# tvlabs/edge264

Hardware: AMD Instinct MI355X
Metric: 1080p frames/s/GPU (bit-exact YUV) + achieved HBM GB/s vs 8 TB/s peak (higher is better)
Workload: dtype u8

## Files before the change

edge264_amd/csrc/e264_dev.h:

```cpp
#ifndef E264_DEV_H
#define E264_DEV_H
#include <stdint.h>
#include <stddef.h>
#include "../../include/edge264_cmd.h"
#include "e264_kernels.h"

#ifndef E264_DEV
#define E264_DEV __device__ __forceinline__
#endif
#ifndef E264_AS_GLOBAL
#define E264_AS_GLOBAL __attribute__((address_space(1)))
#define E264_AS_CONST __attribute__((address_space(4)))
#endif

#ifndef E264_HOST_INTRINSICS
#define E264_FIRST(x) __builtin_amdgcn_readfirstlane(x)
#define E264_BALLOT(x) __ballot(x)
#define E264_ANY(x) __any(x)
#define E264_WG_SYNC() __syncthreads()
#define E264_WG_OR(x) __syncthreads_or(x)
#define E264_SLEEP() __builtin_amdgcn_s_sleep(1)
#define E264_FENCE_ACQUIRE() __builtin_amdgcn_fence(__ATOMIC_ACQUIRE, "workgroup")
#define E264_FENCE_RELEASE() __builtin_amdgcn_fence(__ATOMIC_RELEASE, "workgroup")
#define E264_PROGRESS_STORE(p, v) __hip_atomic_store((p), (v), __ATOMIC_RELAXED, __HIP_MEMORY_SCOPE_WORKGROUP)
#define E264_PROGRESS_LOAD(p) __hip_atomic_load((p), __ATOMIC_RELAXED, __HIP_MEMORY_SCOPE_WORKGROUP)
#define E264_ROW_TAKE(p) __hip_atomic_fetch_add((p), 1, __ATOMIC_RELAXED, __HIP_MEMORY_SCOPE_WORKGROUP)
#define E264_TASK_TAKE(p) atomicAdd((p), 1)
#define E264_SETPRIO(n) __builtin_amdgcn_s_setprio(n)
#define E264_PIN(...) asm volatile("" :: __VA_ARGS__)
#define E264_EMU_DBKP_RAW(L, f, a0)
#define E264_EMU_DBK_STEP(filtered)
#endif
#define E264_MAX_ROWS 1056

namespace {

#if defined(E264_DBK_TIMELINE) || defined(E264_PHASE_TIMING)
__device__ unsigned long long g_phase[32];
__device__ unsigned long long g_timeline[128];
#endif
#ifdef E264_PHASE_TIMING
#define PH_DECL unsigned long long ph_t = __builtin_amdgcn_s_memtime(), ph_acc[14] = {0, 0, 0, 0, 0, 0, 0, 0, 0, 0, 0, 0, 0, 0}
#define PH(k) do { __builtin_amdgcn_sched_barrier(0); unsigned long long t_ = __builtin_amdgcn_s_memtime(); __builtin_amdgcn_s_waitcnt(0xc07f); __builtin_amdgcn_sched_barrier(0); ph_acc[k] += t_ - ph_t; ph_t = t_; } while (0)
#define PH_FLUSH(lane) do { if ((lane) == 0) for (int k_ = 0; k_ < 14; k_++) atomicAdd(&g_phase[k_], ph_acc[k_]); } while (0)
#define PH_FLUSH_DBK(lane) do { if ((lane) == 0) for (int k_ = 0; k_ < 14; k_++) atomicAdd(&g_phase[16 + k_], ph_acc[k_]); } while (0)
#define PH_PARAMS , unsigned long long &ph_t, unsigned long long (&ph_acc)[14]
#define PH_ARGS , ph_t, ph_acc
#else
#define PH_DECL
#define PH(k)
#define PH_FLUSH(lane)
#define PH_FLUSH_DBK(lane)
#define PH_PARAMS
#define PH_ARGS
#endif

E264_DEV int clip3i(int lo, int hi, int v) { return min(max(v, lo), hi); }
E264_DEV int clip255(int v) { return min(max(v, 0), 255); }
E264_DEV int sat16(int v) { return min(max(v, -32768), 32767); }
E264_DEV int w16(int v) { return (int)(int16_t)v; }
#ifdef E264_ABL_NOBH
#define E264_ABL_BH && false
#else
#define E264_ABL_BH
#endif
#ifndef E264_LUMA_PACKED
#define E264_LUMA_PACKED 1
#endif
typedef uint8_t E264_AS_GLOBAL gu8;
typedef uint32_t E264_AS_GLOBAL gu32;
typedef uint16_t E264_AS_GLOBAL gu16;
typedef uint32_t E264_AS_GLOBAL __attribute__((aligned(1))) gu32u;
typedef uint32_t v4u __attribute__((ext_vector_type(4)));
typedef uint32_t v2u __attribute__((ext_vector_type(2)));
typedef v4u E264_AS_GLOBAL __attribute__((aligned(4))) gv4u;
typedef v2u E264_AS_GLOBAL __attribute__((aligned(4))) gv2u;
typedef uint32_t v3u __attribute__((ext_vector_type(3)));
typedef v3u E264_AS_GLOBAL __attribute__((aligned(4))) gv3u;
typedef int16_t E264_AS_GLOBAL gi16;
typedef const E264FrameHdr E264_AS_CONST *chdr_t;
typedef const E264SliceParams E264_AS_CONST *cslice_t;
typedef const E264Mb E264_AS_CONST *cmb_t;
typedef const E264Motion E264_AS_GLOBAL *gmotion_t;
typedef const uint8_t E264_AS_CONST *cu8p;
typedef uint8_t *generic_u8p;
typedef const generic_u8p E264_AS_GLOBAL *gdpb_t;
#ifndef E264_HOST_INTRINSICS
E264_DEV int lane_id() { return (int)(threadIdx.x & 63); }
E264_DEV void wave_sync()
{
	__builtin_amdgcn_fence(__ATOMIC_ACQ_REL, "wavefront");
	__builtin_amdgcn_wave_barrier();
}
#endif
#define lds_load_relaxed(p) E264_PROGRESS_LOAD(p)

__constant__ uint8_t c_BX[16] = {0, 4, 0, 4, 8, 12, 8, 12, 0, 4, 0, 4, 8, 12, 8, 12};
__constant__ uint8_t c_BY[16] = {0, 0, 4, 4, 0, 0, 4, 4, 8, 8, 12, 12, 8, 8, 12, 12};
E264_DEV int BXf(int k) { return ((k & 1) << 2) | ((k & 4) << 1); }
E264_DEV int BYf(int k) { return ((k & 2) << 1) | ((k & 8)); }
E264_DEV int blk_of(int bx, int by) { return (by >> 1) * 8 + (bx >> 1) * 4 + (by & 1) * 2 + (bx & 1); }

E264_DEV int na_byte(uint64_t t, int m) { return (int)(t >> (8 * m)) & 255; }
#define NA4_0 0x12100e0d0b0aull
#define NA4_1 0x1d1917141210ull
E264_DEV int norm4(int m, int pos)
{
	int i = pos >> 2, j = pos & 3;
	const int a = na_byte(NA4_0, m), b = na_byte(NA4_1, m), c = na_byte(0x171412100e0dull, m);
	return (i & j & 1) ? b : ((i | j) & 1) ? c : a;
}
E264_DEV int norm8(int m, int pos)
{
	int i = pos >> 3, j = pos & 7, k;
	const int v0 = na_byte(0x24201c1a1614ull, m), v1 = na_byte(0x201c19171312ull, m), v2 = na_byte(0x3a332d2a2320ull, m);
	const int v3 = na_byte(0x221e1a181513ull, m), v4 = na_byte(0x2e2823211c19ull, m), v5 = na_byte(0x2b26211f1a18ull, m);
	if ((i & 3) == 0 && (j & 3) == 0) k = v0;
	else if (i & j & 1) k = v1;
	else if ((i & 3) == 2 && (j & 3) == 2) k = v2;
	else if (((i & 3) == 0 && (j & 1)) || ((i & 1) && (j & 3) == 0)) k = v3;
	else if (((i & 3) == 0 && (j & 3) == 2) || ((i & 3) == 2 && (j & 3) == 0)) k = v4;
	else k = v5;
	return k;
}

__constant__ uint8_t c_alpha[52] = {0, 0, 0, 0, 0, 0, 0, 0, 0, 0, 0, 0, 0, 0, 0, 0, 4, 4, 5, 6, 7, 8, 9, 10, 12, 13, 15, 17, 20, 22, 25, 28,
	32, 36, 40, 45, 50, 56, 63, 71, 80, 90, 101, 113, 127, 144, 162, 182, 203, 226, 255, 255};
__constant__ uint8_t c_beta[52] = {0, 0, 0, 0, 0, 0, 0, 0, 0, 0, 0, 0, 0, 0, 0, 0, 2, 2, 2, 3, 3, 3, 3, 4, 4, 4, 6, 6, 7, 7, 8, 8,
	9, 9, 10, 10, 11, 11, 12, 12, 13, 13, 14, 14, 15, 15, 16, 16, 17, 17, 18, 18};
__constant__ uint8_t c_tc0[3][52] = {
	{0, 0, 0, 0, 0, 0, 0, 0, 0, 0, 0, 0, 0, 0, 0, 0, 0, 0, 0, 0, 0, 0, 0, 1, 1, 1, 1, 1, 1, 1, 1, 1, 1, 2, 2, 2, 2, 3, 3, 3, 4, 4, 4, 5, 6, 6, 7, 8, 9, 10, 11, 13},
	{0, 0, 0, 0, 0, 0, 0, 0, 0, 0, 0, 0, 0, 0, 0, 0, 0, 0, 0, 0, 0, 1, 1, 1, 1, 1, 1, 1, 1, 1, 1, 2, 2, 2, 2, 3, 3, 3, 4, 4, 5, 5, 6, 7, 8, 8, 10, 11, 12, 13, 15, 17},
	{0, 0, 0, 0, 0, 0, 0, 0, 0, 0, 0, 0, 0, 0, 0, 0, 0, 1, 1, 1, 1, 1, 1, 1, 1, 1, 1, 2, 2, 2, 2, 3, 3, 3, 4, 4, 4, 5, 6, 6, 7, 8, 9, 10, 11, 13, 14, 16, 18, 20, 23, 25}};

#ifndef E264_HOST_INTRINSICS
E264_DEV uint32_t v_perm(uint32_t hi, uint32_t lo, uint32_t sel) { return __builtin_amdgcn_perm(hi, lo, sel); }
E264_DEV uint32_t v_alignbyte(uint32_t hi, uint32_t lo, uint32_t sh) { return __builtin_amdgcn_alignbyte(hi, lo, sh); }
E264_DEV uint32_t v_alignbit(uint32_t hi, uint32_t lo, uint32_t sh) { return __builtin_amdgcn_alignbit(hi, lo, sh); }
E264_DEV uint32_t v_lerp_u8(uint32_t a, uint32_t b, uint32_t c) { return __builtin_amdgcn_lerp(a, b, c); }
E264_DEV int mul24(int a, int b) { return a * b; }
E264_DEV uint32_t v_sat_pk_u8_i16(uint32_t v)
{
	uint32_t r;
	asm("v_sat_pk_u8_i16 %0, %1" : "=v"(r) : "v"(v));
	return r;
}
#endif
typedef short s16x2 __attribute__((ext_vector_type(2)));
E264_DEV s16x2 as_s2(uint32_t v) { return __builtin_bit_cast(s16x2, v); }
E264_DEV uint32_t as_u(s16x2 v) { return __builtin_bit_cast(uint32_t, v); }
template <int I>
E264_DEV s16x2 pair_at(uint32_t hi, uint32_t lo)
{
	return as_s2(v_perm(hi, lo, 0x0c000c00u | (uint32_t)I | (uint32_t)(I + 1) << 16));
}
E264_DEV void pairs9(const uint32_t w[3], s16x2 Q[8])
{
	Q[0] = pair_at<0>(w[1], w[0]); Q[1] = pair_at<1>(w[1], w[0]); Q[2] = pair_at<2>(w[1], w[0]); Q[3] = pair_at<3>(w[1], w[0]);
	Q[4] = pair_at<0>(w[2], w[1]); Q[5] = pair_at<1>(w[2], w[1]); Q[6] = pair_at<2>(w[2], w[1]); Q[7] = pair_at<3>(w[2], w[1]);
}
E264_DEV s16x2 tap6u(s16x2 a, s16x2 b, s16x2 c, s16x2 d, s16x2 e, s16x2 f)
{
	const s16x2 k5 = {-5, -5}, k20 = {20, 20};
	const s16x2 af = as_s2(as_u(a) + as_u(f)), be = as_s2(as_u(b) + as_u(e)), cd = as_s2(as_u(c) + as_u(d));
	return be * k5 + (cd * k20 + af);
}
E264_DEV s16x2 tap6u16(s16x2 a, s16x2 b, s16x2 c, s16x2 d, s16x2 e, s16x2 f)
{
	const s16x2 k5 = {-5, -5}, k20 = {20, 20};
	const s16x2 af = as_s2(as_u(a) + as_u(f) + 0x00100010u), be = as_s2(as_u(b) + as_u(e)), cd = as_s2(as_u(c) + as_u(d));
	return be * k5 + (cd * k20 + af);
}
E264_DEV uint32_t packus4(s16x2 lo, s16x2 hi) { return v_perm(v_sat_pk_u8_i16(as_u(hi)), v_sat_pk_u8_i16(as_u(lo)), 0x05040100u); }
E264_DEV s16x2 tap6p(s16x2 a, s16x2 b, s16x2 c, s16x2 d, s16x2 e, s16x2 f)
{
	const s16x2 k5 = {5, 5}, k20 = {20, 20};
	return (a + f) - (b + e) * k5 + (c + d) * k20;
}
E264_DEV s16x2 centre6p(s16x2 t0, s16x2 t1, s16x2 t2, s16x2 t3, s16x2 t4, s16x2 t5)
{
	const s16x2 s2 = {2, 2}, s6 = {6, 6}, r32 = {32, 32}, z = {0, 0}, m = {255, 255};
	const s16x2 af = t0 + t5, be = t1 + t4, cd = t2 + t3;
	const s16x2 x1 = af - be;
	const s16x2 x2 = (x1 >> s2) + (cd - be);
	const s16x2 x3 = (x2 >> s2) + cd;
	return __builtin_elementwise_min(__builtin_elementwise_max((x3 + r32) >> s6, z), m);
}
E264_DEV s16x2 half5p(s16x2 v)
{
	const s16x2 s5 = {5, 5}, r16 = {16, 16}, z = {0, 0}, m = {255, 255};
	return __builtin_elementwise_min(__builtin_elementwise_max((v + r16) >> s5, z), m);
}
#ifndef E264_HOST_INTRINSICS
E264_DEV uint32_t any_u32() { uint32_t v; asm("" : "=v"(v)); return v; }
#else
E264_DEV uint32_t any_u32() { return 0xa55a5aa5u; }
#endif
E264_DEV uint32_t mot_nmv(uint32_t sub) { return 0x4221u >> (sub * 4) & 15u; }
struct DbkpQuad { v2u a, b; uint32_t c; };
E264_DEV DbkpQuad dbkp_quad_any() { return (DbkpQuad){(v2u){any_u32(), any_u32()}, (v2u){any_u32(), any_u32()}, any_u32()}; }
E264_DEV bool dbkp_list_has(uint32_t h, int l) { return (E264_MOT_UNI(h, l) | (h >> (4 * l) & 15u)) != 0; }
E264_DEV uint32_t dbkp_part_off(uint32_t mot_off, uint32_t h, int l)
{
	uint32_t n0 = 0;
#pragma unroll
	for (int k = 0; k < 4; k++)
		n0 += E264_MOT_USED(h, k) ? 4 + 4 * mot_nmv(E264_MOT_SUB(h, k)) : 0;
	return l ? mot_off + (E264_MOT_UNI(h, 0) ? 8 : n0) : mot_off;
}
E264_DEV DbkpQuad dbkp_fetch_quad(const gu8 *motion, uint32_t pa, uint32_t sub)
{
	DbkpQuad F;
	F.a = *(const gv2u *)(motion + pa);
	F.b = *(const gv2u *)(motion + (pa + (sub == 3 ? 8u : sub ? 4u : 0u)));
	F.c = *(const gu32 *)(motion + (pa + (sub == 3 ? 16u : 0u)));
	return F;
}
E264_DEV uint32_t dbkp_quad_off(uint32_t h, int l, int q)
{
	uint32_t p = 0;
#pragma unroll
	for (int k = 0; k < 3; k++)
		p += (k < q && E264_MOT_USED(h, l * 4 + k)) ? 4 + 4 * mot_nmv(E264_MOT_SUB(h, l * 4 + k)) : 0;
	return p;
}
E264_DEV v4u dbkp_quad_vectors(const DbkpQuad &F, uint32_t sub)
{
	const uint32_t v0 = F.a.y, v1 = F.b.y;
	return (v4u){v0, sub == 3 ? F.b.x : sub == 2 ? v1 : v0, sub == 3 ? v1 : sub == 2 ? v0 : v1, sub == 3 ? F.c : v1};
}
template <int Q0> E264_DEV void dbkp_fetch_list(const gu8 *motion, uint32_t off, uint32_t h, int l, DbkpQuad *F)
{
	const bool uni = E264_MOT_UNI(h, l);
	uint32_t p = 0;
#pragma unroll
	for (int q = 0; q < 4; q++) {
		const bool used = !uni && E264_MOT_USED(h, l * 4 + q);
		const uint32_t sub = used ? E264_MOT_SUB(h, l * 4 + q) : 0;
		if (q >= Q0) {
			const uint32_t pa = off + (used ? p : 0);
#ifdef E264_ABL_DBKP_NOMOT
			F[q - Q0] = (DbkpQuad){(v2u){pa, h}, (v2u){h, pa}, pa};
#else
			F[q - Q0] = dbkp_fetch_quad(motion, pa, sub);
#endif
		}
		p += used ? 4 + 4 * mot_nmv(sub) : 0;
	}
}

struct FrameCtx {
	chdr_t h;
	cslice_t slices;
	cmb_t mbs;
	const gu8 *mbs_g;
	const gu8 *motion;
	const gu8 *payload;
	gdpb_t dpb;
	const generic_u8p *dpb_lds;
	gu8 *cur;
	int W, H;
	int wm, hm;
	int sY, sC;
	uint32_t psY;
	gu8 *dbk;
};

E264_DEV gu8 *plane_base(const FrameCtx &f, gu8 *base, int pl)
{
	return pl == 0 ? base : base + f.psY + (pl == 2 ? (f.sC >> 1) : 0);
}

E264_DEV bool open_frame(FrameCtx &f, const E264Job &job)
{
	const uint8_t *pkt = job.packet;
	chdr_t h = (chdr_t)pkt;
	if (h->magic != E264_MAGIC)
		return false;
	f.h = h;
	f.slices = (cslice_t)(pkt + h->slices_off);
	f.payload = (const gu8 *)(pkt + h->payload_off);
	if (h->version == E264_VERSION) {
		f.mbs = (cmb_t)(pkt + h->mbs_off);
		f.mbs_g = (const gu8 *)(pkt + h->mbs_off);
		f.motion = h->motion_off ? (const gu8 *)(pkt + h->motion_off) : nullptr;
	} else if (h->version - 5u <= 2u && job.expand) {
		f.mbs = (cmb_t)job.expand;
		f.mbs_g = (const gu8 *)job.expand;
		const uint32_t n_compact = *(const uint32_t E264_AS_CONST *)(pkt + h->mbs_off);
		f.motion = (h->motion_off || n_compact) ? (const gu8 *)job.expand + 32u * (uint32_t)h->width_mbs * (uint32_t)h->height_mbs : nullptr;
	} else
		return false;
	f.dpb_lds = nullptr;
	f.dpb = (gdpb_t)job.dpb;
	f.cur = (gu8 *)job.dpb[h->dst_slot];
	f.wm = h->width_mbs; f.hm = h->height_mbs;
	f.W = f.wm * 16; f.H = f.hm * 16;
	f.sY = (int)h->stride_Y; f.sC = (int)h->stride_C;
// ... 8 lines not shown
```

edge264_amd/csrc/e264_pred.h:

```cpp
#ifndef E264_PRED_H
#define E264_PRED_H
#include "e264_dev.h"

namespace {

#ifndef E264_HOST_INTRINSICS
E264_DEV int lds_add(int *p, int v) { return atomicAdd(p, v); }
E264_DEV void lds_or(uint32_t *p, uint32_t v) { atomicOr(p, v); }
#endif

#ifndef E264_HOST_INTRINSICS
E264_DEV uint32_t any_own() { uint32_t v; asm volatile("" : "=v"(v)); return v; }
#else
E264_DEV uint32_t any_own() { return any_u32(); }
#endif
E264_DEV v4u any_v4u() { return (v4u){any_own(), any_own(), any_own(), any_own()}; }

#define PT_W 16
#ifndef E264_PT_H
#define E264_PT_H 4
#endif
#define PT_H E264_PT_H
#define PT_MBS (PT_W * PT_H)
#define PT_NT (PT_MBS * 4)
#define PT_LIST (PT_MBS * 16)

struct __attribute__((aligned(16))) PredLds {
	uint32_t y[PT_H * 16][PT_W * 4];
	uint32_t c[2][PT_H * 8][PT_W * 2];
	uint32_t hdr[PT_MBS][8];
	uint16_t lst[3][PT_LIST];
	uint32_t mvq[4][PT_NT];
	uint32_t refq[PT_NT];
	int cnt[6];
	int rcnt[2];
	uint32_t staged[PT_MBS / 32];
	int any_l1;
	int n_inter, n_uni;
	generic_u8p dpb[E264_MAX_SLOTS];
#ifdef E264_PRED_LDS_PAD
	uint8_t pad[E264_PRED_LDS_PAD];
#endif
};

struct PredTile { int tx0, ty0; };

#define PRED_NO_REF 0xffffffffu
#define PI_SLOT(d) ((d) & 511)
#define PI_SUB(d) ((d) >> 9 & 3)
#define PI_SHAPE(d) ((d) >> 11 & 3)

E264_DEV void pred_phase_setup(PredLds &L, const FrameCtx &f, const PredTile &t, int tid)
{
	const bool rec = tid < PT_MBS * 2, tab = (uint32_t)(tid - PT_MBS * 2) < (uint32_t)E264_MAX_SLOTS;
	const int mb = (tid >> 1) & (PT_MBS - 1), part = tid & 1, k = tab ? tid - PT_MBS * 2 : 0;
	const int mbx = t.tx0 + (mb & (PT_W - 1)), mby = t.ty0 + mb / PT_W;
	const bool in = rec && mbx < f.wm && mby < f.hm;
	v4u r = (v4u){any_u32(), any_u32(), any_u32(), any_u32()};
	if (in) r = *(const gv4u *)(f.mbs_g + (size_t)(mby * f.wm + mbx) * 32 + part * 16);
	v2u d = (v2u){any_u32(), any_u32()};
	static_assert(sizeof(generic_u8p) == 8, "a slot pointer is one 8-byte load");
	if (tab) d = *(const gv2u *)((const gu8 *)f.dpb + k * 8);
	if (rec) *(v4u *)&L.hdr[mb][part * 4] = in ? r : (v4u){0, 0, 0, 0};
	if (tab) *(v2u *)&L.dpb[k] = d;
	if (tid < 6) L.cnt[tid] = 0;
	if (tid < 2) L.rcnt[tid] = 0;
	if (tid < PT_MBS / 32) L.staged[tid] = 0;
	if (tid == 0) { L.any_l1 = 0; L.n_inter = 0; L.n_uni = 0; }
}

static_assert(PT_W == 16, "the bitmap has one 16-bit entry per tile row");
E264_DEV void pred_phase_bitmap(const PredLds &L, const FrameCtx &f, const PredTile &t, int tid)
{
	if (tid >= PT_H || !f.dbk || t.ty0 + tid >= f.hm)
		return;
	uint32_t bits = 0;
#pragma unroll
	for (int i = 0; i < PT_W; i++) {
		const uint32_t d0 = L.hdr[tid * PT_W + i][0];
		const int kind = (d0 >> 8 & E264_MBF_DONE) ? E264_MB_ABSENT : (int)(d0 & 255);
		if (kind == E264_MB_I4x4 || kind == E264_MB_I8x8 || kind == E264_MB_I16x16) bits |= 1u << i;
	}
	gu16 *bitmap = (gu16 *)(f.dbk + E264_BITMAP_OFF(f.wm * f.hm));
	bitmap[(size_t)(t.ty0 + tid) * ((f.wm + 15) >> 4) + (t.tx0 >> 4)] = (uint16_t)bits;
}

E264_DEV int pred_class(uint32_t mv)
{
	const int xF = mv & 3, yF = mv >> 16 & 3;
	if (yF == 0) return xF == 0 ? 0 : 1;
	if (xF == 0) return 2;
	if (xF == 2) return 4;
	return yF == 2 ? 5 : 3;
}
E264_DEV uint16_t *pred_list_slot(PredLds &L, int cls, int idx)
{
	return cls < 3 ? &L.lst[cls][idx] : &L.lst[5 - cls][PT_LIST - 1 - idx];
}
E264_DEV void pred_push(PredLds &L, uint32_t mv, int desc)
{
	const int cls = pred_class(mv);
	*pred_list_slot(L, cls, lds_add(&L.cnt[cls], 1)) = (uint16_t)desc;
}
E264_DEV void pred_phase_classify(PredLds &L, const FrameCtx &f, const PredTile &t, int list, int tid)
{
	const int mb = tid >> 2, q = tid & 3;
	const uint32_t d0 = L.hdr[mb][0];
	const int kind = (d0 >> 8 & E264_MBF_DONE) ? E264_MB_ABSENT : (int)(d0 & 255);
	const bool pcm = list == 0 && kind == E264_MB_PCM, inter = kind == E264_MB_INTER && f.motion;
	const uint32_t mot_off = L.hdr[mb][5], mot_hdr = L.hdr[mb][6];
	const int lo = list ^ 1;
	const bool uni = E264_MOT_UNI(mot_hdr, list), unio = E264_MOT_UNI(mot_hdr, lo);
	const bool used = inter && (uni || E264_MOT_USED(mot_hdr, list * 4 + q));
	const bool usedo = used && (unio || E264_MOT_USED(mot_hdr, lo * 4 + q));
	const uint32_t sub = uni ? 0 : E264_MOT_SUB(mot_hdr, list * 4 + q);
	const int qx = q & 1, qy = q >> 1;
	DbkpQuad F = dbkp_quad_any();
	v2u G = (v2u){any_u32(), any_u32()};
	uint32_t idc = any_u32();
	if (used) {
		F = dbkp_fetch_quad(f.motion, dbkp_part_off(mot_off, mot_hdr, list) + (uni ? 0 : dbkp_quad_off(mot_hdr, list, q)), sub);
		cslice_t s = f.slices + (L.hdr[mb][2] >> 16);
		idc = *(const uint8_t E264_AS_CONST *)&s->weighted_bipred_idc;
	}
	if (usedo) G = *(const gv2u *)(f.motion + (dbkp_part_off(mot_off, mot_hdr, lo) + (unio ? 0 : dbkp_quad_off(mot_hdr, lo, q))));
	v2u py[8];
	uint32_t pc[2][4];
#pragma unroll
	for (int r = 0; r < 8; r++) { py[r] = (v2u){any_own(), any_own()}; pc[r >> 2][r & 3] = any_own(); }
	if (pcm) {
		const gu8 *pl = f.payload + L.hdr[mb][4];
#pragma unroll
		for (int r = 0; r < 8; r++)
			py[r] = *(const gv2u *)(pl + (qy * 8 + r) * 16 + qx * 8);
#pragma unroll
		for (int p = 0; p < 2; p++)
#pragma unroll
			for (int r = 0; r < 4; r++)
				pc[p][r] = *(const gu32 *)(pl + 256 + p * 64 + (qy * 4 + r) * 8 + qx * 4);
	}
	L.refq[tid] = PRED_NO_REF;
	if (list == 0 && (kind == E264_MB_INTER || kind == E264_MB_PCM) && q == 0)
		lds_or(&L.staged[mb >> 5], 1u << (mb & 31));
	if (pcm) {
#pragma unroll
		for (int r = 0; r < 8; r++)
			*(v2u *)&L.y[(mb / PT_W) * 16 + qy * 8 + r][(mb & (PT_W - 1)) * 4 + qx * 2] = py[r];
#pragma unroll
		for (int p = 0; p < 2; p++)
#pragma unroll
			for (int r = 0; r < 4; r++)
				L.c[p][(mb / PT_W) * 8 + qy * 4 + r][(mb & (PT_W - 1)) * 2 + qx] = pc[p][r];
	}
	if (!inter)
		return;
	if (list == 0 && (E264_MOT_UNI(mot_hdr, 1) || E264_MOT_USED(mot_hdr, 4 + q)))
		L.any_l1 = 1;
	if (list == 0 && q == 0) {
		lds_add(&L.n_inter, 1);
		const bool u0 = E264_MOT_UNI(mot_hdr, 0), u1 = E264_MOT_UNI(mot_hdr, 1), any0 = (mot_hdr & 15u) != 0, any1 = (mot_hdr >> 4 & 15u) != 0;
		if ((u0 || !any0) && (u1 || !any1) && (u0 || u1)) lds_add(&L.n_uni, 1);
	}
	if (!used)
		return;
	const uint32_t refword = F.a.x;
	const int pic = (int)(int8_t)refword;
	if (pic < 0)
		return;
	const uint32_t otherref = usedo ? G.x : 0xffffffffu;
// ... 681 lines not shown

E264_DEV void pred_phase_reslist(PredLds &L, int tid)
{
	uint16_t *l4 = &L.lst[0][0], *l8 = &L.lst[2][0];
	const int mb = tid >> 2, q = tid & 3;
	const uint32_t d0 = L.hdr[mb][0], coded = L.hdr[mb][3];
	if ((d0 & 255) != E264_MB_INTER || coded == 0 || (d0 >> 8 & E264_MBF_DONE))
		return;
	const bool t8 = (d0 >> 8) & E264_MBF_T8x8;
	uint32_t bits;
	if (q < 2) bits = t8 ? 0 : coded >> (q * 8) & 255;
	else if (q == 2) bits = (coded & E264_CODED_CHROMA_DC) ? 255 : coded >> 16 & 255;
	else bits = t8 ? ((coded & 1) | (coded >> 3 & 2) | (coded >> 6 & 4) | (coded >> 9 & 8)) : 0;
	while (bits) {
		const int b = __builtin_ctz(bits);
		bits &= bits - 1;
		const uint16_t item = (uint16_t)(mb << 5 | q << 3 | b);
		if (q < 3) l4[lds_add(&L.rcnt[0], 1)] = item;
		else l8[lds_add(&L.rcnt[1], 1)] = item;
	}
}

E264_DEV uint32_t add_res4p(uint32_t px, s16x2 r01, s16x2 r23)
{
	return packus4(pair_at<0>(0, px) + r01, pair_at<2>(0, px) + r23);
}
E264_DEV uint32_t add_res4(uint32_t px, int r0, int r1, int r2, int r3)
{
	const s16x2 r01 = {(short)r0, (short)r1}, r23 = {(short)r2, (short)r3};
	return add_res4p(px, r01, r23);
}

E264_DEV uint32_t sext2(uint32_t w, int hi)
{
	const uint32_t b0 = hi ? w >> 16 : w;
	return ((uint32_t)(int)(int8_t)b0 & 0xffffu) | (uint32_t)(int)(int8_t)(b0 >> 8) << 16;
}

struct ResReq4 { v4u ws, dc, l0, l1; };
struct ResGeo4 { int mb, k, pc, l8, qP; uint32_t d0, coded; bool chroma, has_dc, ac; const gu8 *pl, *co; };
E264_DEV ResGeo4 res_geo4(const PredLds &L, const FrameCtx &f, int item)
{
	ResGeo4 g;
	const int b = item & 31;
	g.mb = item >> 5;
	const uint32_t d0 = L.hdr[g.mb][0], d1 = L.hdr[g.mb][1], coded = L.hdr[g.mb][3];
	const bool t8 = (d0 >> 8) & E264_MBF_T8x8;
	g.d0 = d0; g.coded = coded;
	g.pl = f.payload + L.hdr[g.mb][4];
	const gu8 *pl = (coded & E264_CODED_CHROMA_DC) ? g.pl + 16 : g.pl;
	g.chroma = b >= 16;
	g.k = b & 15;
	g.pc = (g.k >> 2) & 1;
	g.l8 = (d0 >> 8 & E264_MBF_LEV8) ? 1 : 0;
	const int lumab = (t8 ? __builtin_popcount(coded & 0x1111) * 128 : __builtin_popcount(coded & 0xffff) * 32) >> g.l8;
	g.co = g.chroma ? pl + lumab + ((__builtin_popcount((coded >> 16) & ((1u << g.k) - 1)) * 32) >> g.l8)
	                : pl + ((__builtin_popcount(coded & ((1u << g.k) - 1)) * 32) >> g.l8);
	g.qP = g.chroma ? (g.pc ? (int)(d1 & 255) : (int)(d0 >> 24)) : (int)(d0 >> 16 & 255);
	g.has_dc = g.chroma && (coded & E264_CODED_CHROMA_DC);
	g.ac = g.chroma ? (coded >> (16 + g.k) & 1) : true;
	return g;
}
E264_DEV void res_req4(const PredLds &L, const FrameCtx &f, const ResGeo4 &g, ResReq4 &R)
{
	cslice_t s = f.slices + (L.hdr[g.mb][2] >> 16);
	const int wl = g.chroma ? 4 + g.pc : 3;
	R.ws = *(const gv4u *)((const gu8 *)s + offsetof(E264SliceParams, weightScale4x4) + wl * 16);
	R.dc = any_v4u(); R.l0 = any_v4u(); R.l1 = any_v4u();
	if (g.has_dc) R.dc = *(const gv4u *)g.pl;
	if (g.ac) R.l0 = *(const gv4u *)g.co;
	if (g.ac && !g.l8) R.l1 = *(const gv4u *)(g.co + 16);
}
E264_DEV void res_item4(PredLds &L, const ResGeo4 &g, const ResReq4 &R)
{
	const int mb = g.mb, k = g.k, pc = g.pc;
	const bool chroma = g.chroma, has_dc = g.has_dc, ac = g.ac;
	const int sh = g.qP / 6, m = g.qP - sh * 6;
	const uint32_t ws[4] = {R.ws.x, R.ws.y, R.ws.z, R.ws.w};
	const int na = na_byte(NA4_0, m), nb = na_byte(NA4_1, m), nc = na_byte(0x171412100e0dull, m);
	int dc = 0;
	if (has_dc) {
		const int hs = pc * 16;
		const int c0 = (int)(int16_t)(R.dc.x >> hs), c2 = (int)(int16_t)(R.dc.y >> hs), c4 = (int)(int16_t)(R.dc.z >> hs), c6 = (int)(int16_t)(R.dc.w >> hs), n = k & 3;
		const int v = n == 0 ? c0 + c4 + c2 + c6 : n == 1 ? c0 - c4 + c2 - c6 : n == 2 ? c0 + c4 - c2 - c6 : c0 - c4 - c2 + c6;
		const int LS = (int)((ws[0] & 255u) * (uint32_t)na) << sh;
		dc = (int)((uint32_t)v * (uint32_t)LS) >> 5;
	}
	int r[4][4];
	if (ac) {
		uint32_t cw[8];
		if (g.l8) {
			const uint32_t w[4] = {R.l0.x, R.l0.y, R.l0.z, R.l0.w};
#pragma unroll
			for (int i = 0; i < 4; i++) { cw[2 * i] = sext2(w[i], 0); cw[2 * i + 1] = sext2(w[i], 1); }
		} else {
			cw[0] = R.l0.x; cw[1] = R.l0.y; cw[2] = R.l0.z; cw[3] = R.l0.w; cw[4] = R.l1.x; cw[5] = R.l1.y; cw[6] = R.l1.z; cw[7] = R.l1.w;
		}
		int tt[4][4];
#pragma unroll
		for (int y = 0; y < 4; y++) {
			int d[4];
#pragma unroll
			for (int x = 0; x < 4; x++) {
				const int pos = x * 4 + y;
				const int lev = (int)(int16_t)(cw[pos >> 1] >> ((pos & 1) * 16));
				const int wsb = (int)(ws[pos >> 2] >> ((pos & 3) * 8) & 255u);
				const int nrm = (x & y & 1) ? nb : ((x | y) & 1) ? nc : na;
				d[x] = (int)(((uint32_t)(lev * (wsb * nrm)) << sh) + 8u) >> 4;
			}
			if (chroma && y == 0) d[0] = dc;
			const int e0 = d[0] + d[2], e1 = d[0] - d[2], e2 = (d[1] >> 1) - d[3], e3 = (d[3] >> 1) + d[1];
			const int add = y == 0 ? 32 : 0;
			tt[0][y] = e0 + e3 + add; tt[1][y] = e1 + e2 + add; tt[2][y] = e1 - e2 + add; tt[3][y] = e0 - e3 + add;
		}
#pragma unroll
		for (int x = 0; x < 4; x++) {
			const int f0 = tt[x][0], f1 = tt[x][1], f2 = tt[x][2], f3 = tt[x][3];
			const int g0 = f0 + f2, g1 = f0 - f2, g2 = (f1 >> 1) - f3, g3 = (f3 >> 1) + f1;
			r[0][x] = sat16((g0 + g3) >> 6); r[1][x] = sat16((g1 + g2) >> 6); r[2][x] = sat16((g1 - g2) >> 6); r[3][x] = sat16((g0 - g3) >> 6);
		}
	} else {
		const int v = (int)(int16_t)((dc + 32) >> 6);
#pragma unroll
		for (int y = 0; y < 4; y++)
#pragma unroll
			for (int x = 0; x < 4; x++) r[y][x] = v;
	}
	uint32_t *px;
	int stride;
	if (chroma) { px = &L.c[pc][(mb / PT_W) * 8 + ((k >> 1) & 1) * 4][(mb & (PT_W - 1)) * 2 + (k & 1)]; stride = PT_W * 2; }
	else { px = &L.y[(mb / PT_W) * 16 + BYf(k)][(mb & (PT_W - 1)) * 4 + (BXf(k) >> 2)]; stride = PT_W * 4; }
#pragma unroll
	for (int y = 0; y < 4; y++)
		px[y * stride] = add_res4(px[y * stride], r[y][0], r[y][1], r[y][2], r[y][3]);
}

E264_DEV void idct8_1dp(s16x2 d[8])
{
	const s16x2 s1 = {1, 1}, s2 = {2, 2};
	const s16x2 d0 = d[0], d1 = d[1], d2 = d[2], d3 = d[3], d4 = d[4], d5 = d[5], d6 = d[6], d7 = d[7];
	const s16x2 e0 = d0 + d4;
	const s16x2 e1 = d5 - d3 - ((d7 >> s1) + d7);
	const s16x2 e2 = d0 - d4;
	const s16x2 e3 = d1 + d7 - ((d3 >> s1) + d3);
	const s16x2 e4 = (d2 >> s1) - d6;
	const s16x2 e5 = d7 - d1 + ((d5 >> s1) + d5);
	const s16x2 e6 = (d6 >> s1) + d2;
	const s16x2 e7 = d3 + d5 + ((d1 >> s1) + d1);
	const s16x2 f0 = e0 + e6, f1 = (e7 >> s2) + e1, f2 = e2 + e4, f3 = (e5 >> s2) + e3;
	const s16x2 f4 = e2 - e4, f5 = (e3 >> s2) - e5, f6 = e0 - e6, f7 = e7 - (e1 >> s2);
	d[0] = f0 + f7; d[1] = f2 + f5; d[2] = f4 + f3; d[3] = f6 + f1;
	d[4] = f6 - f1; d[5] = f4 - f3; d[6] = f2 - f5; d[7] = f0 - f7;
}
struct ResReq8 { v4u ws[4], lv[8]; };
struct ResGeo8 { int mb, bq, l8, qP; const gu8 *co; };
E264_DEV ResGeo8 res_geo8(const PredLds &L, const FrameCtx &f, int item)
{
	ResGeo8 g;
	g.mb = item >> 5; g.bq = (item & 31) - 24;
	const uint32_t d0 = L.hdr[g.mb][0], coded = L.hdr[g.mb][3];
	const gu8 *pl = f.payload + L.hdr[g.mb][4];
	if (coded & E264_CODED_CHROMA_DC) pl += 16;
	g.l8 = (d0 >> 8 & E264_MBF_LEV8) ? 1 : 0;
	g.co = pl + ((__builtin_popcount(coded & 0x1111 & ((1u << (g.bq * 4)) - 1)) * 128) >> g.l8);
	g.qP = (int)(d0 >> 16 & 255);
	return g;
}
E264_DEV void res_req8(const PredLds &L, const FrameCtx &f, const ResGeo8 &g, ResReq8 &R)
{
	cslice_t s = f.slices + (L.hdr[g.mb][2] >> 16);
	const gu8 *wsp = (const gu8 *)s + offsetof(E264SliceParams, weightScale8x8) + 64;
#pragma unroll
	for (int i = 0; i < 4; i++) {
		R.ws[i] = *(const gv4u *)(wsp + i * 16);
		R.lv[i] = *(const gv4u *)(g.co + i * 16);
		R.lv[4 + i] = any_v4u();
	}
	if (!g.l8) {
#pragma unroll
		for (int i = 0; i < 4; i++) R.lv[4 + i] = *(const gv4u *)(g.co + 64 + i * 16);
	}
}
E264_DEV void res_item8(PredLds &L, const ResGeo8 &g, const ResReq8 &R)
{
	const int mb = g.mb, bq = g.bq;
	const int qP = g.qP, div = qP / 6, m = qP - div * 6;
	const int shl = max(div - 6, 0), shr = max(6 - div, 0), rnd = div < 6 ? 1 << (5 - div) : 0;
	const int lo = div < 6 ? -32768 : (int)0x80000000, hi = div < 6 ? 32767 : 0x7fffffff;
	uint32_t lev8[8][4];
	if (g.l8) {
#pragma unroll
		for (int i = 0; i < 8; i++) {
			const v4u v = R.lv[i >> 1];
			const uint32_t a = (i & 1) ? v.z : v.x, b = (i & 1) ? v.w : v.y;
			lev8[i][0] = sext2(a, 0); lev8[i][1] = sext2(a, 1); lev8[i][2] = sext2(b, 0); lev8[i][3] = sext2(b, 1);
		}
	} else {
#pragma unroll
		for (int i = 0; i < 8; i++) { lev8[i][0] = R.lv[i].x; lev8[i][1] = R.lv[i].y; lev8[i][2] = R.lv[i].z; lev8[i][3] = R.lv[i].w; }
	}
	s16x2 t[8][4];
#pragma unroll
	for (int i = 0; i < 8; i++) {
		const uint32_t *cw = lev8[i];
		const v4u wv = R.ws[i >> 1];
		const uint32_t ww[2] = {(i & 1) ? wv.z : wv.x, (i & 1) ? wv.w : wv.y};
#pragma unroll
		for (int jp = 0; jp < 4; jp++) {
			int dq[2];
#pragma unroll
			for (int h = 0; h < 2; h++) {
				const int j = jp * 2 + h, pos = i * 8 + j;
				const int lev = (int)(int16_t)(cw[jp] >> (h * 16));
				const int LS = (int)(ww[j >> 2] >> ((j & 3) * 8) & 255u) * norm8(m, pos);
				dq[h] = min(max((lev * (int)(int16_t)(LS << shl) + rnd) >> shr, lo), hi);
			}
			const s16x2 v = {(short)dq[0], (short)dq[1]};
			t[i][jp] = v;
		}
	}
#pragma unroll
	for (int jp = 0; jp < 4; jp++) {
		s16x2 d[8];
#pragma unroll
		for (int i = 0; i < 8; i++) d[i] = t[i][jp];
		idct8_1dp(d);
#pragma unroll
		for (int i = 0; i < 8; i++) t[i][jp] = d[i];
	}
	s16x2 u[8][4];
#pragma unroll
	for (int ip = 0; ip < 4; ip++)
#pragma unroll
		for (int jp = 0; jp < 4; jp++) {
			const uint32_t a = as_u(t[2 * ip][jp]), b = as_u(t[2 * ip + 1][jp]);
			u[2 * jp][ip] = as_s2(v_perm(b, a, 0x05040100u));
			u[2 * jp + 1][ip] = as_s2(v_perm(b, a, 0x07060302u));
		}
	const s16x2 r32 = {32, 32}, s6 = {6, 6};
#pragma unroll
	for (int ip = 0; ip < 4; ip++) {
		s16x2 d[8];
#pragma unroll
		for (int j = 0; j < 8; j++) d[j] = u[j][ip];
		d[0] = d[0] + r32;
		idct8_1dp(d);
#pragma unroll
		for (int j = 0; j < 8; j++) u[j][ip] = d[j] >> s6;
	}
	uint32_t *px = &L.y[(mb / PT_W) * 16 + (bq >> 1) * 8][(mb & (PT_W - 1)) * 4 + (bq & 1) * 2];
#pragma unroll
	for (int j = 0; j < 8; j++) {
#pragma unroll
		for (int w = 0; w < 2; w++) {
			px[j * PT_W * 4 + w] = add_res4p(px[j * PT_W * 4 + w], u[j][2 * w], u[j][2 * w + 1]);
		}
	}
}
E264_DEV void pred_phase_residual(PredLds &L, const FrameCtx &f, int tid)
{
	const int n4 = L.rcnt[0], n8 = L.rcnt[1];
	const uint16_t *l4 = &L.lst[0][0], *l8 = &L.lst[2][0];
#ifdef E264_PRED_RES8_FIRST_WAVES
	const int p8 = tid;
#else
	const int p8 = PT_NT - 1 - tid;
#endif
	const bool has4 = tid < n4, has8 = p8 < n8;
	const ResGeo4 g4 = res_geo4(L, f, has4 ? l4[tid] : 0);
	const ResGeo8 g8 = res_geo8(L, f, has8 ? l8[p8] : 24);
	ResReq4 R4 = {any_v4u(), any_v4u(), any_v4u(), any_v4u()};
	ResReq8 R8;
#pragma unroll
	for (int i = 0; i < 8; i++) { R8.ws[i >> 1] = any_v4u(); R8.lv[i] = any_v4u(); }
	if (has4) res_req4(L, f, g4, R4);
	if (has8) res_req8(L, f, g8, R8);
	if (has4) res_item4(L, g4, R4);
	if (has8) res_item8(L, g8, R8);
}
static_assert(PT_MBS * 4 <= PT_NT, "the 8x8 blocks of a tile are one pass");
E264_DEV void pred_phase_residual_more(PredLds &L, const FrameCtx &f, int k, int tid)
{
	const int p = k * PT_NT + tid;
	if (p >= L.rcnt[0])
		return;
	const uint16_t *l4 = &L.lst[0][0];
	const ResGeo4 g4 = res_geo4(L, f, l4[p]);
	ResReq4 R4;
	res_req4(L, f, g4, R4);
	res_item4(L, g4, R4);
}
E264_DEV int pred_residual_passes(const PredLds &L)
{
	return (L.rcnt[0] + PT_NT - 1) / PT_NT;
}

E264_DEV void pred_phase_flush(const PredLds &L, const FrameCtx &f, const PredTile &t, int tid)
{
	gu8 *Yb = f.cur + (size_t)(t.ty0 * 16) * f.sY + t.tx0 * 16;
	for (int i = tid; i < PT_H * 16 * PT_W; i += PT_NT) {
		const int row = i / PT_W, c = i & (PT_W - 1), mb = (row >> 4) * PT_W + c;
		if (L.staged[mb >> 5] >> (mb & 31) & 1)
			*(gv4u *)(Yb + (size_t)row * f.sY + c * 16) = *(const v4u *)&L.y[row][c * 4];
	}
	for (int i = tid; i < 2 * PT_H * 8 * (PT_W / 2); i += PT_NT) {
		const int pc = i / (PT_H * 8 * (PT_W / 2)), rem = i - pc * (PT_H * 8 * (PT_W / 2));
		const int row = rem / (PT_W / 2), c = rem & (PT_W / 2 - 1), mb = (row >> 3) * PT_W + c * 2;
		const uint32_t st = L.staged[mb >> 5] >> (mb & 31) & 3;
		gu8 *dst = plane_base(f, f.cur, 1 + pc) + (size_t)(t.ty0 * 8 + row) * f.sC + t.tx0 * 8 + c * 16;
		const v4u v = *(const v4u *)&L.c[pc][row][c * 4];
		if (st == 3) *(gv4u *)dst = v;
		else if (st == 1) { const v2u h = {v.x, v.y}; *(gv2u *)dst = h; }
		else if (st == 2) { const v2u h = {v.z, v.w}; *(gv2u *)(dst + 8) = h; }
	}
}

#ifdef E264_WG_SYNC
E264_DEV void pred_kernel_body(PredLds &L, const E264Job &job, const int bx, const int tid)
{
	FrameCtx f;
	if (!open_frame(f, job))
		return;
	const int ntx = (f.wm + PT_W - 1) / PT_W, nty = (f.hm + PT_H - 1) / PT_H;
	if (bx >= ntx * nty)
		return;
	const PredTile t = {(bx % ntx) * PT_W, (bx / ntx) * PT_H};
	PH_DECL;
	pred_phase_setup(L, f, t, tid);
	PH(0);
	E264_WG_SYNC();
	pred_phase_bitmap(L, f, t, tid);
	{
		const int kind = tid < PT_MBS ? (int)(L.hdr[tid][0] & 255) : 0;
		if (!E264_WG_OR(kind == E264_MB_INTER || kind == E264_MB_PCM))
			return;
	}
	PH(1);
	pred_phase_classify(L, f, t, 0, tid);
	PH(2);
	E264_WG_SYNC();
	PH(3);
	pred_phase_items(L, f, t, 0, tid);
	PH(4);
	E264_WG_SYNC();
	PH(5);
	if (L.any_l1) {
		pred_phase_reset(L, tid);
		E264_WG_SYNC();
		pred_phase_classify(L, f, t, 1, tid);
		E264_WG_SYNC();
		pred_phase_items(L, f, t, 1, tid);
		E264_WG_SYNC();
	}
	PH(6);
	pred_phase_reslist(L, tid);
	PH(7);
	E264_WG_SYNC();
	PH(8);
	pred_phase_residual(L, f, tid);
	for (int k = 1, n = pred_residual_passes(L); k < n; k++) {
		E264_WG_SYNC();
		pred_phase_residual_more(L, f, k, tid);
	}
	PH(9);
	E264_WG_SYNC();
	PH(10);
	pred_phase_flush(L, f, t, tid);
	PH(11);
	PH_FLUSH(tid & 63);
}
#endif
}
#endif
```

Baseline: 95640.

## Split each 8x8 residual IDCT across a lane pair using DPP swaps

Each 8x8 luma residual block is now handled by two adjacent lanes, each dequantising and transforming half the block. The lanes exchange intermediate halves through DPP quad-permute moves between the dequant, row-pass and column-pass stages. The goal is to halve per-lane register pressure and the serial critical path of the 8x8 transform, at the cost of permute instructions and possibly extra residual passes, since 8x8 blocks now take two threads each. The 4x4 and 8x8 residual phases are merged into one function that is called per pass.

```diff
diff --git a/edge264_amd/csrc/e264_dev.h b/edge264_amd/csrc/e264_dev.h
--- a/edge264_amd/csrc/e264_dev.h
+++ b/edge264_amd/csrc/e264_dev.h
@@ -144,6 +144,22 @@
 	uint32_t r;
 	asm("v_sat_pk_u8_i16 %0, %1" : "=v"(r) : "v"(v));
 	return r;
+}
+#endif
+#ifndef E264_HOST_INTRINSICS
+template <int N> E264_DEV void pair_swap(uint32_t (&v)[N], int tid)
+{
+#pragma unroll
+	for (int i = 0; i < N; i++) v[i] = (uint32_t)__builtin_amdgcn_mov_dpp((int)v[i], 0xb1, 0xf, 0xf, true);
+}
+#elif defined(E264_WG_SYNC)
+template <int N> E264_DEV void pair_swap(uint32_t (&v)[N], int tid)
+{
+	static uint32_t s[1024][N];
+	for (int i = 0; i < N; i++) s[tid][i] = v[i];
+	E264_WG_SYNC();
+	for (int i = 0; i < N; i++) v[i] = s[tid ^ 1][i];
+	E264_WG_SYNC();
 }
 #endif
 typedef short s16x2 __attribute__((ext_vector_type(2)));
diff --git a/edge264_amd/csrc/e264_pred.h b/edge264_amd/csrc/e264_pred.h
--- a/edge264_amd/csrc/e264_pred.h
+++ b/edge264_amd/csrc/e264_pred.h
@@ -15,6 +15,11 @@
 E264_DEV uint32_t any_own() { return any_u32(); }
 #endif
 E264_DEV v4u any_v4u() { return (v4u){any_own(), any_own(), any_own(), any_own()}; }
+#ifndef E264_HOST_INTRINSICS
+E264_DEV int here(int v) { asm volatile("" : "+v"(v)); return v; }
+#else
+E264_DEV int here(int v) { return v; }
+#endif
 
 #define PT_W 16
 #ifndef E264_PT_H
@@ -1002,148 +1007,157 @@
 	d[0] = f0 + f7; d[1] = f2 + f5; d[2] = f4 + f3; d[3] = f6 + f1;
 	d[4] = f6 - f1; d[5] = f4 - f3; d[6] = f2 - f5; d[7] = f0 - f7;
 }
-struct ResReq8 { v4u ws[4], lv[8]; };
-struct ResGeo8 { int mb, bq, l8, qP; const gu8 *co; };
-E264_DEV ResGeo8 res_geo8(const PredLds &L, const FrameCtx &f, int item)
+struct ResReq8 { v4u ws[2], lv[4]; };
+struct ResGeo8 { int mb, bq, l8, qP, h; const gu8 *co; };
+E264_DEV ResGeo8 res_geo8(const PredLds &L, const FrameCtx &f, int item, int h)
 {
 	ResGeo8 g;
-	g.mb = item >> 5; g.bq = (item & 31) - 24;
+	g.mb = item >> 5; g.bq = (item & 31) - 24; g.h = h;
 	const uint32_t d0 = L.hdr[g.mb][0], coded = L.hdr[g.mb][3];
 	const gu8 *pl = f.payload + L.hdr[g.mb][4];
 	if (coded & E264_CODED_CHROMA_DC) pl += 16;
 	g.l8 = (d0 >> 8 & E264_MBF_LEV8) ? 1 : 0;
-	g.co = pl + ((__builtin_popcount(coded & 0x1111 & ((1u << (g.bq * 4)) - 1)) * 128) >> g.l8);
+	g.co = pl + ((__builtin_popcount(coded & 0x1111 & ((1u << (g.bq * 4)) - 1)) * 128 + h * 64) >> g.l8);
 	g.qP = (int)(d0 >> 16 & 255);
 	return g;
 }
 E264_DEV void res_req8(const PredLds &L, const FrameCtx &f, const ResGeo8 &g, ResReq8 &R)
 {
 	cslice_t s = f.slices + (L.hdr[g.mb][2] >> 16);
-	const gu8 *wsp = (const gu8 *)s + offsetof(E264SliceParams, weightScale8x8) + 64;
-#pragma unroll
-	for (int i = 0; i < 4; i++) {
+	const gu8 *wsp = (const gu8 *)s + offsetof(E264SliceParams, weightScale8x8) + 64 + g.h * 32;
+#pragma unroll
+	for (int i = 0; i < 2; i++) {
 		R.ws[i] = *(const gv4u *)(wsp + i * 16);
 		R.lv[i] = *(const gv4u *)(g.co + i * 16);
-		R.lv[4 + i] = any_v4u();
+		R.lv[2 + i] = any_v4u();
 	}
 	if (!g.l8) {
 #pragma unroll
-		for (int i = 0; i < 4; i++) R.lv[4 + i] = *(const gv4u *)(g.co + 64 + i * 16);
-	}
-}
-E264_DEV void res_item8(PredLds &L, const ResGeo8 &g, const ResReq8 &R)
-{
-	const int mb = g.mb, bq = g.bq;
+		for (int i = 0; i < 2; i++) R.lv[2 + i] = *(const gv4u *)(g.co + 32 + i * 16);
+	}
+}
+struct Res8 { s16x2 x[4][2], y[4][2]; uint32_t sw[8]; };
+E264_DEV void res8_give(Res8 &S, int h)
+{
+#pragma unroll
+	for (int i = 0; i < 8; i++) {
+		const uint32_t x = as_u(S.x[i >> 1][i & 1]), y = as_u(S.y[i >> 1][i & 1]);
+		S.sw[i] = h ? x : y;
+	}
+}
+E264_DEV void res8_take(const Res8 &S, int h, int q, s16x2 d[8])
+{
+#pragma unroll
+	for (int i = 0; i < 4; i++) {
+		const uint32_t r = S.sw[i * 2 + q], x = as_u(S.x[i][q]), y = as_u(S.y[i][q]);
+		d[i] = as_s2(h ? r : x);
+		d[4 + i] = as_s2(h ? y : r);
+	}
+}
+E264_DEV void res8_dequant(const ResGeo8 &g, const ResReq8 &R, Res8 &S)
+{
 	const int qP = g.qP, div = qP / 6, m = qP - div * 6;
 	const int shl = max(div - 6, 0), shr = max(6 - div, 0), rnd = div < 6 ? 1 << (5 - div) : 0;
 	const int lo = div < 6 ? -32768 : (int)0x80000000, hi = div < 6 ? 32767 : 0x7fffffff;
-	uint32_t lev8[8][4];
-	if (g.l8) {
-#pragma unroll
-		for (int i = 0; i < 8; i++) {
-			const v4u v = R.lv[i >> 1];
-			const uint32_t a = (i & 1) ? v.z : v.x, b = (i & 1) ? v.w : v.y;
-			lev8[i][0] = sext2(a, 0); lev8[i][1] = sext2(a, 1); lev8[i][2] = sext2(b, 0); lev8[i][3] = sext2(b, 1);
-		}
-	} else {
-#pragma unroll
-		for (int i = 0; i < 8; i++) { lev8[i][0] = R.lv[i].x; lev8[i][1] = R.lv[i].y; lev8[i][2] = R.lv[i].z; lev8[i][3] = R.lv[i].w; }
-	}
-	s16x2 t[8][4];
-#pragma unroll
-	for (int i = 0; i < 8; i++) {
-		const uint32_t *cw = lev8[i];
-		const v4u wv = R.ws[i >> 1];
-		const uint32_t ww[2] = {(i & 1) ? wv.z : wv.x, (i & 1) ? wv.w : wv.y};
+#pragma unroll
+	for (int ii = 0; ii < 4; ii++) {
+		const v4u wv = R.ws[ii >> 1];
+		uint32_t cw[4];
+		if (g.l8) {
+			const v4u lv = R.lv[ii >> 1];
+			const uint32_t a = (ii & 1) ? lv.z : lv.x, b = (ii & 1) ? lv.w : lv.y;
+			cw[0] = sext2(a, 0); cw[1] = sext2(a, 1); cw[2] = sext2(b, 0); cw[3] = sext2(b, 1);
+		} else {
+			cw[0] = R.lv[ii].x; cw[1] = R.lv[ii].y; cw[2] = R.lv[ii].z; cw[3] = R.lv[ii].w;
+		}
+		const uint32_t ww[2] = {(ii & 1) ? wv.z : wv.x, (ii & 1) ? wv.w : wv.y};
 #pragma unroll
 		for (int jp = 0; jp < 4; jp++) {
 			int dq[2];
 #pragma unroll
-			for (int h = 0; h < 2; h++) {
-				const int j = jp * 2 + h, pos = i * 8 + j;
-				const int lev = (int)(int16_t)(cw[jp] >> (h * 16));
+			for (int hh = 0; hh < 2; hh++) {
+				const int j = jp * 2 + hh, pos = ii * 8 + j;
+				const int lev = (int)(int16_t)(cw[jp] >> (hh * 16));
 				const int LS = (int)(ww[j >> 2] >> ((j & 3) * 8) & 255u) * norm8(m, pos);
-				dq[h] = min(max((lev * (int)(int16_t)(LS << shl) + rnd) >> shr, lo), hi);
+				dq[hh] = min(max((lev * (int)(int16_t)(LS << shl) + rnd) >> shr, lo), hi);
 			}
 			const s16x2 v = {(short)dq[0], (short)dq[1]};
-			t[i][jp] = v;
-		}
-	}
-#pragma unroll
-	for (int jp = 0; jp < 4; jp++) {
+			if (jp < 2) S.x[ii][jp] = v;
+			else S.y[ii][jp - 2] = v;
+		}
+	}
+	res8_give(S, g.h);
+}
+E264_DEV void res8_pass1(const ResGeo8 &g, Res8 &S)
+{
+	s16x2 t[8][2];
+#pragma unroll
+	for (int q = 0; q < 2; q++) {
 		s16x2 d[8];
-#pragma unroll
-		for (int i = 0; i < 8; i++) d[i] = t[i][jp];
+		res8_take(S, g.h, q, d);
 		idct8_1dp(d);
 #pragma unroll
-		for (int i = 0; i < 8; i++) t[i][jp] = d[i];
-	}
-	s16x2 u[8][4];
+		for (int i = 0; i < 8; i++) t[i][q] = d[i];
+	}
 #pragma unroll
 	for (int ip = 0; ip < 4; ip++)
 #pragma unroll
-		for (int jp = 0; jp < 4; jp++) {
-			const uint32_t a = as_u(t[2 * ip][jp]), b = as_u(t[2 * ip + 1][jp]);
-			u[2 * jp][ip] = as_s2(v_perm(b, a, 0x05040100u));
-			u[2 * jp + 1][ip] = as_s2(v_perm(b, a, 0x07060302u));
-		}
+		for (int q = 0; q < 2; q++) {
+			const uint32_t a = as_u(t[2 * ip][q]), b = as_u(t[2 * ip + 1][q]);
+			const s16x2 e = as_s2(v_perm(b, a, 0x05040100u)), o = as_s2(v_perm(b, a, 0x07060302u));
+			if (ip < 2) { S.x[2 * q][ip] = e; S.x[2 * q + 1][ip] = o; }
+			else { S.y[2 * q][ip - 2] = e; S.y[2 * q + 1][ip - 2] = o; }
+		}
+	res8_give(S, g.h);
+}
+E264_DEV void res8_pass2(PredLds &L, const ResGeo8 &g, const Res8 &S)
+{
 	const s16x2 r32 = {32, 32}, s6 = {6, 6};
-#pragma unroll
-	for (int ip = 0; ip < 4; ip++) {
+	s16x2 u[8][2];
+#pragma unroll
+	for (int p = 0; p < 2; p++) {
 		s16x2 d[8];
-#pragma unroll
-		for (int j = 0; j < 8; j++) d[j] = u[j][ip];
+		res8_take(S, g.h, p, d);
 		d[0] = d[0] + r32;
 		idct8_1dp(d);
 #pragma unroll
-		for (int j = 0; j < 8; j++) u[j][ip] = d[j] >> s6;
-	}
-	uint32_t *px = &L.y[(mb / PT_W) * 16 + (bq >> 1) * 8][(mb & (PT_W - 1)) * 4 + (bq & 1) * 2];
-#pragma unroll
-	for (int j = 0; j < 8; j++) {
-#pragma unroll
-		for (int w = 0; w < 2; w++) {
-			px[j * PT_W * 4 + w] = add_res4p(px[j * PT_W * 4 + w], u[j][2 * w], u[j][2 * w + 1]);
-		}
-	}
-}
-E264_DEV void pred_phase_residual(PredLds &L, const FrameCtx &f, int tid)
-{
+		for (int j = 0; j < 8; j++) u[j][p] = d[j] >> s6;
+	}
+	uint32_t *px = &L.y[(g.mb / PT_W) * 16 + (g.bq >> 1) * 8][(g.mb & (PT_W - 1)) * 4 + (g.bq & 1) * 2 + g.h];
+#pragma unroll
+	for (int j = 0; j < 8; j++) px[j * PT_W * 4] = add_res4p(px[j * PT_W * 4], u[j][0], u[j][1]);
+}
+#ifdef E264_WG_SYNC
+E264_DEV void pred_phase_residual(PredLds &L, const FrameCtx &f, int k, int tid0)
+{
+	const int tid = here(tid0);
 	const int n4 = L.rcnt[0], n8 = L.rcnt[1];
 	const uint16_t *l4 = &L.lst[0][0], *l8 = &L.lst[2][0];
-#ifdef E264_PRED_RES8_FIRST_WAVES
-	const int p8 = tid;
-#else
-	const int p8 = PT_NT - 1 - tid;
-#endif
-	const bool has4 = tid < n4, has8 = p8 < n8;
-	const ResGeo4 g4 = res_geo4(L, f, has4 ? l4[tid] : 0);
-	const ResGeo8 g8 = res_geo8(L, f, has8 ? l8[p8] : 24);
+	const int p4 = k * PT_NT + tid, p8 = k * (PT_NT / 2) + ((PT_NT - 1 - tid) >> 1);
+	const bool has4 = p4 < n4, has8 = p8 < n8;
+	const ResGeo4 g4 = res_geo4(L, f, has4 ? l4[p4] : 0);
+	const ResGeo8 g8 = res_geo8(L, f, has8 ? l8[p8] : 24, tid & 1);
 	ResReq4 R4 = {any_v4u(), any_v4u(), any_v4u(), any_v4u()};
 	ResReq8 R8;
 #pragma unroll
-	for (int i = 0; i < 8; i++) { R8.ws[i >> 1] = any_v4u(); R8.lv[i] = any_v4u(); }
+	for (int i = 0; i < 4; i++) { R8.ws[i >> 1] = any_v4u(); R8.lv[i] = any_v4u(); }
 	if (has4) res_req4(L, f, g4, R4);
 	if (has8) res_req8(L, f, g8, R8);
 	if (has4) res_item4(L, g4, R4);
-	if (has8) res_item8(L, g8, R8);
-}
-static_assert(PT_MBS * 4 <= PT_NT, "the 8x8 blocks of a tile are one pass");
-E264_DEV void pred_phase_residual_more(PredLds &L, const FrameCtx &f, int k, int tid)
-{
-	const int p = k * PT_NT + tid;
-	if (p >= L.rcnt[0])
-		return;
-	const uint16_t *l4 = &L.lst[0][0];
-	const ResGeo4 g4 = res_geo4(L, f, l4[p]);
-	ResReq4 R4;
-	res_req4(L, f, g4, R4);
-	res_item4(L, g4, R4);
+	Res8 S;
+#pragma unroll
+	for (int i = 0; i < 8; i++) S.sw[i] = any_own();
+	if (has8) res8_dequant(g8, R8, S);
+	pair_swap(S.sw, tid);
+	if (has8) res8_pass1(g8, S);
+	pair_swap(S.sw, tid);
+	if (has8) res8_pass2(L, g8, S);
 }
 E264_DEV int pred_residual_passes(const PredLds &L)
 {
-	return (L.rcnt[0] + PT_NT - 1) / PT_NT;
-}
+	return max((L.rcnt[0] + PT_NT - 1) / PT_NT, (L.rcnt[1] + PT_NT / 2 - 1) / (PT_NT / 2));
+}
+#endif
 
 E264_DEV void pred_phase_flush(const PredLds &L, const FrameCtx &f, const PredTile &t, int tid)
 {
@@ -1207,10 +1221,10 @@
 	PH(7);
 	E264_WG_SYNC();
 	PH(8);
-	pred_phase_residual(L, f, tid);
+	pred_phase_residual(L, f, 0, tid);
 	for (int k = 1, n = pred_residual_passes(L); k < n; k++) {
 		E264_WG_SYNC();
-		pred_phase_residual_more(L, f, k, tid);
+		pred_phase_residual(L, f, k, tid);
 	}
 	PH(9);
 	E264_WG_SYNC();
```

After: 96560, median of 6. About the same (+1.0%).
